# tianhao-stan-wu/LLA-MPC

Hardware: AMD Instinct MI355X
Metric: model-rollouts/sec (N_models x H steps) per control tick; wall-clock per plan() call (higher is better)
Workload: dtype f64

## Files before the change

### __graft_entry__.py

```python
import os
import subprocess
import sys

REPO = os.path.dirname(os.path.abspath(__file__))
PKG_ROOT = os.path.join(REPO, "lla-mpc_amd")
CSRC = os.path.join(PKG_ROOT, "csrc")
LIB = os.path.join(PKG_ROOT, "llampc", "_lib", "libllampc_hip.so")


def _paths():
    for p in (REPO, PKG_ROOT):
        if p not in sys.path:
            sys.path.insert(0, p)


SOURCES = ("capi.hip", "capi_xchg.hip", "capi_ctl.hip", "capi_nlp.hip", "kernels.hip", "ctl.hip", "plan_rk4_l4.hip",
           "plan_rk4_l2.hip", "plan_rk4_l1.hip", "plan_euler.hip", "plan_rk6.hip", "nlp.hip")


def build() -> None:
    hipcc = os.environ.get("HIPCC", "/opt/rocm/bin/hipcc")
    os.makedirs(os.path.dirname(LIB), exist_ok=True)
    objdir = os.path.join(PKG_ROOT, "build")
    os.makedirs(objdir, exist_ok=True)
    flags = ["--offload-arch=gfx950", "-O3", "-std=c++17", "-fPIC", "-mllvm", "-disable-machine-licm",
             f"-I{os.path.join(REPO, 'include')}", "-Wall", "-Wno-unused-result"]
    jobs = max(1, min(len(SOURCES), int(os.environ.get("MAX_JOBS", os.cpu_count() or 4))))
    objs, pending = [], []
    for src in SOURCES:
        obj = os.path.join(objdir, src.replace(".hip", ".o"))
        objs.append(obj)
        pending.append([hipcc, *flags, "-c", "-o", obj, os.path.join(CSRC, src)])
    running = []
    while pending or running:
        while pending and len(running) < jobs:
            cmd = pending.pop(0)
            running.append((cmd, subprocess.Popen(cmd)))
        cmd, p = running.pop(0)
        if p.wait() != 0:
            for _, q in running:
                q.wait()
            raise subprocess.CalledProcessError(p.returncode, cmd)
    subprocess.run([hipcc, "--offload-arch=gfx950", "-shared", "-fPIC", "-o", LIB, *objs], check=True)
    _paths()
    import llampc
    import llampc.mpc
    from llampc import _native
    _native.load()


def smoke() -> None:
    _paths()
    import numpy as np
    from llampc.mpc import ModelBank, generate_bank, plan
    from oracle import llampc_oracle as O

    N, W, K, H, C, Ts = 512, 3, 5, 20, 4, 0.02
    bank_p = generate_bank(N, seed=0)
    p = O.orca_params()
    shared = {k: p[k] for k in ("lf", "lr", "mass", "Iz", "Cm1", "Cm2", "Cr0", "Cr2")}
    rng = np.random.RandomState(5)
    xs = [np.array([0.5, -1.0, -0.6, 1.8, 0.05, 0.4])]
    us = rng.uniform([0.2, -0.2], [0.8, 0.2], size=(W + 2, 2))
    v_true = O.Vehicle.from_params(p, Df=p["Df"] * 0.8, Dr=p["Dr"] * 0.8)
    for k in range(W + 1):
# ... 29 lines not shown
```

### lla-mpc_amd/csrc/lookahead_dev.hpp

```cpp
#pragma once
#include "dev_stamps.hpp"
#include "dev_wave.hpp"
#include "raceline.hpp"
#include "rollout_dev.hpp"

namespace llampc {

template <int NW = kWaves>
__device__ __forceinline__ void la_publish(const LookaheadLaunch& a, int blk, const Scratch& sc, int par,
                                           double v, int64_t key, int nf) {
  static_assert(NW == kWaves || NW == 8, "4- or 8-wave blocks");
  wave_pick_nl64(v, key);
  const int nfw = wave_sum(nf);
  double* sv = sc.sv + 4 * par;
  int64_t* si = sc.si + 4 * par;
  if ((threadIdx.x & 63) == 0) {
    sv[threadIdx.x >> 6] = v;
    si[threadIdx.x >> 6] = key;
    sc.sn[threadIdx.x >> 6] = nfw;
  }
  __syncthreads();
  if (threadIdx.x == 0) {
    int nfs = sc.sn[0];
#pragma unroll
    for (int w = 1; w < NW; ++w) {
      const bool t = (int)(si[w] != kNoIndex) & (int)less_bf<0>(sv[w], si[w], v, key);
      v = t ? sv[w] : v;
      key = t ? si[w] : key;
      nfs += sc.sn[w];
    }
    if (a.poll) {
      uint64_t* r = a.blk_tag + 5 * (int64_t)blk;
      const uint64_t vb = (uint64_t)__double_as_longlong(v), kb = (uint64_t)key;
      st_wt(&r[0], tag_word(a.seq, (uint32_t)(vb >> 32)));
      st_wt(&r[1], tag_word(a.seq, (uint32_t)vb));
      st_wt(&r[2], tag_word(a.seq, (uint32_t)(kb >> 32)));
      st_wt(&r[3], tag_word(a.seq, (uint32_t)kb));
      st_wt(&r[4], tag_word(a.seq, (uint32_t)nfs));
    } else {
      st_wt(&a.pv[blk], v);
      st_wt(&a.pidx[blk], key);
      st_wt(&a.pnf[blk], nfs);
    }
  }
}

template <int INTEG, bool STAGE, int LPM, int XM, int WQ = 0>
__device__ __forceinline__ void lookahead_block(const LookaheadLaunch& a, int blk, int G, int cpl,
                                                unsigned char* smem, const Scratch& sc) {
  LA_STAMP(blk, 0);
  constexpr int BT = wq_threads(WQ);
  double* sx = reinterpret_cast<double*>(smem + kScratchBytes);
  double* su = sx + 2 * (a.H + 1);
  const int H = a.H, C = a.C;
  const int sub = threadIdx.x % LPM;
  const int cl = threadIdx.x / LPM;
  const int g = cl & (G - 1);
  const int64_t n = (int64_t)blk * (kBlock / (G * LPM)) + cl / G;
  const bool live = n < a.n;
  const int mpb = kBlock / (G * LPM);
  const int soff = (XM && mpb < kBlock) ? mpb : 0;
  Tire t{};
  if (!WQ && live) t = load_tire(a.params, a.n, n);
  double x0[6];
#pragma unroll
  for (int m = 0; m < 6; ++m) x0[m] = a.x0[m];
  double* rl_knots = su + (STAGE ? kStageW * C * H : 0);
  double* rl_xy = rl_knots + a.rl.n + kKnotPad;
  if (XM) {
    const int nk = a.rl.n, nseg = a.rl.n - 1, nxy = 8 * nseg;
    const double* gk = a.rl.knots;
    const double* gmu = a.rl.mus;
    double* rl_mus = rl_xy + nxy;
    copy_lds<4>(rl_knots, nk, [&](int e) { return gk[e]; });
    copy_lds<24>(rl_xy, nxy + a.rl.M, [&](int e) {
      const double* p = e < nxy ? gk + nk + e : gmu + (e - nxy);
      return *p;
    });
    if ((int)threadIdx.x < kKnotPad) rl_knots[nk + threadIdx.x] = __builtin_inf();
    const double s0 = a.xref[0];
    const double L = gk[nseg];
    const double adv = window_adv(a.xref[1], a.xref[2], a.Ts, H, a.rl.vmax);
    const bool bounded = adv < L && s0 >= 0.0 && s0 < L;
    double te = s0 + adv;
    if (te >= L) te -= L;
    __syncthreads();
    RL_STAMP(blk, 0);
    int* rl_sel = reinterpret_cast<int*>(sx);
    for (int i = threadIdx.x; i < nseg; i += kBlock) {
      const double ki = rl_knots[i], kn = rl_knots[i + 1];
      const bool last = i == nseg - 1;
      if ((i == 0 || ki <= s0) && (last || !(kn <= s0))) rl_sel[0] = i;
      if ((i == 0 || ki <= te) && (last || !(kn <= te))) rl_sel[1] = i;
    }
    __syncthreads();
    SpeedWin sw{nullptr, 0, 0};
    const int seg0 = rl_sel[0];
    {
      const int lo = seg0, l2 = rl_sel[1];
// ... 19 lines not shown
        const int drow = kBlock / W, dj = kBlock - drow * W, rows = a.rl.M * 4;
        copy_lds<24>(wl, tot, [&](int) {
          int sg = lo + j;
          if (sg >= nseg) sg -= nseg;
          const double v = gsp[(size_t)(row < rows ? row : rows - 1) * nseg + sg];
          row += drow;
          j += dj;
          if (j >= W) {
            j -= W;
            ++row;
          }
          return v;
        });
        __syncthreads();
      }
    }
    RL_STAMP(blk, 1);
    const int64_t m = (int64_t)blk * mpb + threadIdx.x;
    if ((int)threadIdx.x < mpb && m < a.n) {
      const double mu = (a.params[2 * a.n + m] + a.params[5 * a.n + m]) / (9.81 * a.veh.mass);
      const RacelineK rl = a.rl;
      RaceRef rr;
      rr.init(rl, rl_knots, rl_mus, mu, a.xref[0], a.xref[1], a.xref[2], a.Ts, seg0);
      double2* out = reinterpret_cast<double2*>(a.xref_pm + m * 2 * H);
      for (int k = 0; k < H; ++k) {
        double xr, yr;
        rr.step(rl, rl_knots, rl_xy, sw, xr, yr);
        out[k] = make_double2(xr, yr);
      }
    }
    RL_STAMP(blk, 2);
    __threadfence_block();
    RL_STAMP(blk, 3);
  } else {
    for (int e = threadIdx.x; e <= H; e += BT) {
      sx[2 * e] = a.xref[e];
      sx[2 * e + 1] = a.xref[(H + 1) + e];
    }
  }
  fm::FmK K0;
  if constexpr (!XM) K0 = fm::FmK::load<kLeanLA && INTEG == 0>();
  if (STAGE) {
    const fm::FmK K = [&] {
      if constexpr (XM) return fm::FmK::load();
      else return K0;
    }();
    const FusedK fq0 = make_fused(a.veh, make_stage<1>(a.veh, Tire{}, 0), a.Ts, scaled_yaw(LPM));
    for (int e = (int)threadIdx.x - soff; e < C * H; e += BT - soff) {
      if (e < 0) break;
      const int c = e / H, k = e - c * H;
      const double dl = a.U[2 * e + 1];
      double sd, cd;
      if (fm::sincos_fast_ok(dl)) fm::sincos_fast(dl, &sd, &cd, K);
      else LL_SINCOS(dl, &sd, &cd);
      double* o = su + kStageW * (k * C + c);
      const double ua = a.U[2 * e];
      const double p0 = k ? a.U[2 * e - 2] : a.uprev[0], p1 = k ? a.U[2 * e - 1] : a.uprev[1];
      const double d0 = ua - p0, d1 = dl - p1;
      if (INTEG == 0) {
        const FusedIn fi = fused_in(fq0, Input{ua, dl, sd, cd});
        o[0] = fi.F0;
        o[1] = fi.F1;
        o[2] = fi.hmsd;
        o[3] = fi.hmcd;
        o[4] = fi.c5a;
        o[5] = dl;
      } else {
        o[0] = ua;
        o[1] = dl;
        o[2] = sd;
        o[3] = cd;
      }
      o[6] = act_term(a.cost, d0, d1);
      o[7] = (!a.cost.enforce || input_feasible(a.cost, ua, dl, d0, d1)) ? 1.0 : 0.0;
    }
  }
  __syncthreads();

  CostK q = a.cost;
  VehK veh = a.veh;
  double Ts = a.Ts;
  for (int m = 0; m < 4; ++m) {
    pin_vgpr(q.Q[m]);
    pin_vgpr(q.R[m]);
    pin_vgpr(q.P[m]);
  }
  for (int m = 0; m < 2; ++m) {
    pin_vgpr(q.umin[m]);
    pin_vgpr(q.umax[m]);
    pin_vgpr(q.dmax[m]);
  }
  pin_vgpr(veh.lf);
  pin_vgpr(veh.lr);
  pin_vgpr(veh.mass);
  pin_vgpr(veh.inv_mass);
  pin_vgpr(veh.inv_Iz);
  pin_vgpr(veh.Cm1);
  pin_vgpr(veh.Cm2);
  pin_vgpr(veh.Cr0);
  pin_vgpr(veh.Cr2);
  pin_vgpr(Ts);
  const double up0 = a.uprev[0], up1 = a.uprev[1];

  double bv = __builtin_nan("");
  int64_t bc = kNoIndex;
  int nf = 0;
  LA_STAMP(blk, 1);
  constexpr bool kSplit = (INTEG == 0 && LPM == 4);
  constexpr unsigned kRF = (STAGE ? kRStage : 0u) | (XM ? kRXm : 0u);
  constexpr unsigned kRSplitQ = kSplit ? kRSplit : 0u;
  const bool diagQP = a.cost.Q[1] == 0.0 && a.cost.Q[2] == 0.0 && a.cost.P[1] == 0.0 && a.cost.P[2] == 0.0;
  if constexpr (WQ) {
    static_assert(LPM == 1 && XM == 0, "work queue: LPM 1, shared xref");
    const int mpw = 64 / G;
    const int64_t units = (a.n + mpw - 1) / mpw;
    const int lm = (int)(threadIdx.x & 63) / G;
    uint32_t zoff;
    asm volatile("v_mov_b32 %0, 0" : "=v"(zoff));
    auto issue = [&](uint32_t off) -> uint64_t {
      uint64_t v = 0;
      if ((threadIdx.x & 63) == 0)
        v = __hip_atomic_fetch_add(a.wq + off, (uint64_t)1, __ATOMIC_RELAXED, __HIP_MEMORY_SCOPE_AGENT);
      return v;
    };
    auto take = [&](uint64_t v) -> int64_t {
      const uint32_t lo = (uint32_t)__builtin_amdgcn_readlane((int)(uint32_t)v, 0);
      const uint32_t hi = (uint32_t)__builtin_amdgcn_readlane((int)(uint32_t)(v >> 32), 0);
      return (int64_t)(((uint64_t)hi << 32) | lo);
    };
    double vacc = __builtin_nan("");
    int64_t kacc = kNoIndex;
    int nfacc = 0;
    const fm::FmK K = K0;
#ifdef LLAMPC_STAMPS
    int ju = 0;
// ... 44 lines not shown
        }
      }
      WQ_STAMP(blk, ju, 2);
      const int64_t un = take(nxt);
      if (lv && g == 0) {
        if (a.poll) {
          st_wt(&a.la_tag[nm], tag_word(a.seq, (uint32_t)(__double_as_longlong(mv) >> 32)));
          st_wt(&a.la_tag[a.n + nm], tag_word(a.seq, (uint32_t)__double_as_longlong(mv)));
          st_wt(&a.la_tag[2 * a.n + nm], tag_word(a.seq, (uint32_t)(int32_t)mc));
        } else {
          st_wt(&a.best_cand[nm], (int32_t)mc);
          st_wt(&a.best_cost[nm], mv);
        }
        if (mc != kNoIndex) {
          const int64_t key = (a.goff + nm) * C + mc;
          if (less_bf<0>(mv, key, vacc, kacc)) {
            vacc = mv;
            kacc = key;
          }
        }
      }
      WQ_STAMP(blk, ju, 3);
#ifdef LLAMPC_STAMPS
      ++ju;
#endif
      u = un;
    }
    LA_STAMP(blk, 2);
    la_publish<BT / 64>(a, blk, sc, 0, vacc, kacc, nfacc);
    LA_STAMP(blk, 3);
    return;
  }
  if (live) {
    constexpr bool kScaled = (INTEG == 0 && scaled_yaw(LPM));
    StageK sk = make_stage<LPM>(veh, t, sub, INTEG == 0 ? Ts : 1.0);
    if (kScaled) sk.ch[0].lw = sk.ch[0].lw / Ts;
    if (kScaled && LPM == 1) sk.ch[1].lw = sk.ch[1].lw / Ts;
    if (kScaled && LPM == 4 && sub >= 2) {
      sk.ch[0].lw = 0.0;
      sk.ch[0].sg = 0.0;
      sk.ch[0].B = 0.0;
      sk.ch[0].nsB = 0.0;
    }
    const FusedK fq = make_fused(veh, sk, Ts, kScaled);
    const fm::FmK K = [&] {
      if constexpr (XM) return fm::FmK::load<kLeanLA && INTEG == 0>();
      else return K0;
    }();
    for (int j = 0; j < cpl; ++j) {
      const int c = g + j * G;
      if (c >= C) break;
      bool bad = false;
      double J;
      if (kSplit && diagQP)
        J = rollout<INTEG, LPM, kRF | kRFast | kRSplitQ>(a, c, n, x0, sx, su, veh, t, sk, q, Ts, up0, up1, K, fq, bad);
      else
        J = rollout<INTEG, LPM, kRF | kRFast>(a, c, n, x0, sx, su, veh, t, sk, q, Ts, up0, up1, K, fq, bad);
      if (LPM == 2) {
        const int bi = bad;
        bad = __builtin_amdgcn_mov_dpp(bi, kPair0, 0xF, 0xF, false) |
              __builtin_amdgcn_mov_dpp(bi, kPair1, 0xF, 0xF, false);
      } else if (LPM == 4) {
        int bi = bad;
        bi |= __builtin_amdgcn_mov_dpp(bi, kQuadX1, 0xF, 0xF, false);
        bi |= __builtin_amdgcn_mov_dpp(bi, kQuadX2, 0xF, 0xF, false);
        bad = bi;
      }
      if (__builtin_expect(__any(bad), 0)) {
        bool unused = false;
        if (bad) J = rollout<INTEG, LPM, kRF>(a, c, n, x0, sx, su, veh, t, sk, q, Ts, up0, up1, K, fq, unused);
      }
      if (sub == 0) {
        if (a.cost_out) a.cost_out[n * C + c] = J;
        nf += !isfinite(J);
      }
      if (less_nan_last(J, c, bv, bc)) {
        bv = J;
// ... 54 lines not shown
```

### lla-mpc_amd/csrc/plan_dev.hpp

```cpp
#pragma once
#include <algorithm>

#include "final_dev.hpp"
#include "lookahead_dev.hpp"
#include "lookback_dev.hpp"
#include "peer_dev.hpp"

namespace llampc {

template <int INTEG, bool STAGE, int LPM, int XM, bool PX = false, int WQ = 0>
__device__ __forceinline__ void plan_body(const LookbackLaunch& lb, const LookaheadLaunch& la,
                                          const FinalLaunch& fin, int G, int cpl) {
  extern __shared__ __attribute__((aligned(16))) unsigned char smem[];
  const Scratch sc(smem);
  int* flag = reinterpret_cast<int*>(smem + kFlagOff);
  const bool is_lb = (int)blockIdx.x < fin.nb_lb;
  const int lb_blk = (int)blockIdx.x, la_blk = (int)blockIdx.x - fin.nb_lb;
  if constexpr (wq_threads(WQ) > kBlock) {
    if (is_lb && threadIdx.x >= kBlock) return;
  }
  if (is_lb) {
    lookback_block(lb, lb_blk, sc);
    if (!ticket_last(&fin.tickets[0], (unsigned)fin.nb_lb, flag)) return;
    if (fin.full) {
      lb_final(fin, smem);
      if (fin.host_tag) __threadfence_system();
    }
    if (fin.poll) {
      __syncthreads();
      final_poll(fin, sc);
      if constexpr (PX) peer_finish(fin, smem);
      return;
    }
  } else {
    lookahead_block<INTEG, STAGE, LPM, XM, WQ>(la, la_blk, G, cpl, smem, sc);
    if (fin.poll) return;
    if constexpr (wq_threads(WQ) > kBlock) {
      if (threadIdx.x >= kBlock) return;
    }
  }
  const unsigned expected = (unsigned)fin.nb_la + (fin.nb_lb > 0 ? 1u : 0u);
  if (!ticket_last(&fin.tickets[1], expected, flag)) return;
  final_select(fin, sc);
  if constexpr (PX) peer_finish(fin, smem);
}

template <int INTEG, bool STAGE, int LPM, int XM, bool PX = false, int WQ = 0>
__global__ __launch_bounds__(wq_threads(WQ)) void plan_kernel(LookbackLaunch lb, LookaheadLaunch la,
                                                      FinalLaunch fin, int G, int cpl) {
  plan_body<INTEG, STAGE, LPM, XM, PX, WQ>(lb, la, fin, G, cpl);
}

template <int LPM>
__global__ __launch_bounds__(kBlock) void plan_kernel_inl(LookbackLaunch lb, LookaheadLaunch la,
                                                          FinalLaunch fin, int G, int cpl,
                                                          InlinePack pk) {
  const double* v = pk.v;
  lb.x_prev = v;
  lb.u_prev = v + 6;
  lb.x_now = v + 8;
  la.x0 = v + 8;
  la.uprev = v + 14;
  la.xref = v + 16;
  la.U = v + 16 + 2 * (la.H + 1);
  plan_body<0, true, LPM, 0>(lb, la, fin, G, cpl);
}

constexpr size_t kOneBlockPerCuLds = 82 * 1024;

template <int INTEG, bool STAGE, int PX, int WQ>
static void launch_plan_wq(const LookbackLaunch& lb, const LookaheadLaunch& la, const FinalLaunch& f,
                           int G, int cpl, size_t lds, hipStream_t s) {
  allow_lds(plan_kernel<INTEG, STAGE, 1, 0, PX, WQ>);
  hipLaunchKernelGGL((plan_kernel<INTEG, STAGE, 1, 0, PX, WQ>), dim3(f.nb_lb + f.nb_la), dim3(wq_threads(WQ)),
                     lds, s, lb, la, f, G, cpl);
}

template <int INTEG, bool STAGE, int LPM>
static void launch_plan_t(const LookbackLaunch& lb, const LookaheadLaunch& la, const FinalLaunch& f,
                          int G, int cpl, size_t lds, hipStream_t s, int wq = 0) {
  lds = std::max(lds, kOneBlockPerCuLds);
  if constexpr (INTEG == LLAMPC_RK4 && LPM == 1) {
    if (wq) {
      if constexpr (STAGE) {
        if (wq == 2) {
          if (f.px_G) launch_plan_wq<INTEG, STAGE, 1, 2>(lb, la, f, G, cpl, lds, s);
          else launch_plan_wq<INTEG, STAGE, 0, 2>(lb, la, f, G, cpl, lds, s);
          return;
        }
      }
      if (f.px_G) launch_plan_wq<INTEG, STAGE, 1, 1>(lb, la, f, G, cpl, lds, s);
      else launch_plan_wq<INTEG, STAGE, 0, 1>(lb, la, f, G, cpl, lds, s);
      return;
    }
  }
  if constexpr (INTEG == LLAMPC_RK4) {
    if (f.px_G) {
      allow_lds(plan_kernel<INTEG, STAGE, LPM, 0, true>);
      hipLaunchKernelGGL((plan_kernel<INTEG, STAGE, LPM, 0, true>), dim3(f.nb_lb + f.nb_la), dim3(kBlock), lds,
                         s, lb, la, f, G, cpl);
      return;
    }
  }
  if (la.xref_mode == LLAMPC_XREF_RACELINE) {
    allow_lds(plan_kernel<INTEG, STAGE, LPM, 1>);
    hipLaunchKernelGGL((plan_kernel<INTEG, STAGE, LPM, 1>), dim3(f.nb_lb + f.nb_la), dim3(kBlock), lds, s,
                       lb, la, f, G, cpl);
  } else {
    allow_lds(plan_kernel<INTEG, STAGE, LPM, 0>);
    hipLaunchKernelGGL((plan_kernel<INTEG, STAGE, LPM, 0>), dim3(f.nb_lb + f.nb_la), dim3(kBlock), lds, s,
                       lb, la, f, G, cpl);
  }
}

template <int LPM>
static void launch_plan_inl(const LookbackLaunch& lb, const LookaheadLaunch& la, const FinalLaunch& f,
                            int G, int cpl, size_t lds, hipStream_t s, const InlinePack& pk) {
  lds = std::max(lds, kOneBlockPerCuLds);
  allow_lds(plan_kernel_inl<LPM>);
  hipLaunchKernelGGL((plan_kernel_inl<LPM>), dim3(f.nb_lb + f.nb_la), dim3(kBlock), lds, s, lb, la, f,
                     G, cpl, pk);
}

template <int INTEG, int LPM>
void launch_plan_group(const LookbackLaunch& lb, const LookaheadLaunch& la, const FinalLaunch& f, int G,
                       int cpl, bool stage, size_t lds, hipStream_t s, int wq) {
  if (stage) launch_plan_t<INTEG, true, LPM>(lb, la, f, G, cpl, lds, s, wq);
  else launch_plan_t<INTEG, false, LPM>(lb, la, f, G, cpl, lds, s, wq);
}

template <int LPM>
void launch_plan_inline_group(const LookbackLaunch& lb, const LookaheadLaunch& la, const FinalLaunch& f,
                              int G, int cpl, size_t lds, hipStream_t s, const InlinePack& pk) {
  launch_plan_inl<LPM>(lb, la, f, G, cpl, lds, s, pk);
}

}
```

### lla-mpc_amd/csrc/dev_wave.hpp

```cpp
#pragma once
#include <hip/hip_runtime.h>
#include <stdint.h>

#include "kernels.hpp"

namespace llampc {

namespace {

template <int NAN_FIRST>
__device__ __forceinline__ bool kless(double av, int64_t ai, double bv, int64_t bi) {
  return NAN_FIRST ? less_nan_first(av, ai, bv, bi) : less_nan_last(av, ai, bv, bi);
}

constexpr int kDppXor1 = 0xB1, kDppXor2 = 0x4E, kDppRor4 = 0x124, kDppRor8 = 0x128;
template <int CTRL>
__device__ __forceinline__ int dpp_i(int x) {
  return __builtin_amdgcn_update_dpp(x, x, CTRL, 0xF, 0xF, false);
}
template <int CTRL>
__device__ __forceinline__ double dpp_d(double v) {
  return __hiloint2double(dpp_i<CTRL>(__double2hiint(v)), dpp_i<CTRL>(__double2loint(v)));
}
template <int CTRL>
__device__ __forceinline__ int64_t dpp_l(int64_t v) {
  const uint64_t u = (uint64_t)v;
  const uint64_t lo = (uint32_t)dpp_i<CTRL>((int)(uint32_t)u), hi = (uint32_t)dpp_i<CTRL>((int)(u >> 32));
  return (int64_t)(lo | (hi << 32));
}
__device__ __forceinline__ double readlane_d(double v, int l) {
  return __hiloint2double(__builtin_amdgcn_readlane(__double2hiint(v), l),
                          __builtin_amdgcn_readlane(__double2loint(v), l));
}
__device__ __forceinline__ int64_t readlane_l(int64_t v, int l) {
  const uint64_t u = (uint64_t)v;
  const uint64_t lo = (uint32_t)__builtin_amdgcn_readlane((int)(uint32_t)u, l);
  const uint64_t hi = (uint32_t)__builtin_amdgcn_readlane((int)(u >> 32), l);
  return (int64_t)(lo | (hi << 32));
}

template <int NAN_FIRST, int CTRL>
__device__ __forceinline__ void min_step(double& v, int64_t& i) {
  const double ov = dpp_d<CTRL>(v);
  const int64_t oi = dpp_l<CTRL>(i);
  if (kless<NAN_FIRST>(ov, oi, v, i)) {
    v = ov;
    i = oi;
  }
}

template <int NAN_FIRST>
__device__ __forceinline__ void wave_min(double& v, int64_t& i) {
  min_step<NAN_FIRST, kDppXor1>(v, i);
  min_step<NAN_FIRST, kDppXor2>(v, i);
  min_step<NAN_FIRST, kDppRor4>(v, i);
  min_step<NAN_FIRST, kDppRor8>(v, i);
  double bv = readlane_d(v, 0);
  int64_t bi = readlane_l(i, 0);
#pragma unroll
  for (int r = 16; r < 64; r += 16) {
    const double rv = readlane_d(v, r);
    const int64_t ri = readlane_l(i, r);
    if (kless<NAN_FIRST>(rv, ri, bv, bi)) {
      bv = rv;
      bi = ri;
// ... 60 lines not shown
  int64_t q = (int64_t)((double)key / dc);
  q += (int64_t)((double)(key - q * C) / dc);
  int64_t r = key - q * C;
  if (r < 0) {
    q -= 1;
    r += C;
  } else if (r >= C) {
    q += 1;
    r -= C;
  }
  m = q;
  c = (int32_t)r;
}

__device__ __forceinline__ uint64_t tag_word(uint32_t seq, uint32_t payload) {
  return ((uint64_t)seq << 32) | payload;
}
__device__ __forceinline__ bool tag_ok(uint64_t w, uint32_t seq) { return (uint32_t)(w >> 32) == seq; }
__device__ __forceinline__ uint64_t join_words(uint64_t hi, uint64_t lo) {
  return ((uint64_t)(uint32_t)hi << 32) | (uint32_t)lo;
}

__device__ __forceinline__ int wave_sum(int x) {
  x += dpp_i<kDppXor1>(x);
  x += dpp_i<kDppXor2>(x);
  x += dpp_i<kDppRor4>(x);
  x += dpp_i<kDppRor8>(x);
  return __builtin_amdgcn_readlane(x, 0) + __builtin_amdgcn_readlane(x, 16) +
         __builtin_amdgcn_readlane(x, 32) + __builtin_amdgcn_readlane(x, 48);
}

__device__ __forceinline__ void pin_vgpr(double& x) { asm volatile("" : "+v"(x)); }

}

constexpr int kScratchBytes = 192;
constexpr int kFlagOff = 160;
constexpr int kLateOff = 168;
constexpr int kStageW = 8;
constexpr int kRankBytes = 64 * 8 + 64 * 4 + 256;
constexpr int kWaves = kBlock / 64;
constexpr int kListsPerLane = 8;

struct Scratch {
  double* sv;
  int64_t* si;
  int32_t* sn;
  __device__ explicit Scratch(unsigned char* smem)
      : sv(reinterpret_cast<double*>(smem)),
        si(reinterpret_cast<int64_t*>(smem + 64)),
        sn(reinterpret_cast<int32_t*>(smem + 128)) {}
};

template <int NAN_FIRST>
__device__ __forceinline__ void block_min1(double& v, int64_t& i, const Scratch& s, int& par) {
  wave_min<NAN_FIRST>(v, i);
  double* sv = s.sv + 4 * par;
  int64_t* si = s.si + 4 * par;
  par ^= 1;
  if ((threadIdx.x & 63) == 0) {
    sv[threadIdx.x >> 6] = v;
    si[threadIdx.x >> 6] = i;
  }
  __syncthreads();
  v = sv[0];
  i = si[0];
// ... 22 lines not shown
```

Before: 8.347 billion.

## Preload hot kernel arguments and issue early loads ahead of lookahead setup

The plan kernel signature is reordered so the most-used scalars and pointers come first, and a compiler flag enables kernarg preloading into SGPRs for the plan sources; the remaining launch structs are read through the kernarg segment pointer. Lookahead blocks now issue their tire, x0, uprev and first control loads before the main setup, prefetch the next staged control input inside the stage loop, and defer the xref writes to LDS until after staging. The goal is to hide global-load latency at kernel start and cut kernarg fetch cost, at the price of extra register pressure and reliance on a backend-specific LLVM option.

```diff
diff --git a/__graft_entry__.py b/__graft_entry__.py
--- a/__graft_entry__.py
+++ b/__graft_entry__.py
@@ -30,7 +30,8 @@
     for src in SOURCES:
         obj = os.path.join(objdir, src.replace(".hip", ".o"))
         objs.append(obj)
-        pending.append([hipcc, *flags, "-c", "-o", obj, os.path.join(CSRC, src)])
+        plan = ["-mllvm", "-amdgpu-kernarg-preload-count=16"] if src.startswith("plan_") else []
+        pending.append([hipcc, *flags, *plan, "-c", "-o", obj, os.path.join(CSRC, src)])
     running = []
     while pending or running:
         while pending and len(running) < jobs:
diff --git a/lla-mpc_amd/csrc/lookahead_dev.hpp b/lla-mpc_amd/csrc/lookahead_dev.hpp
--- a/lla-mpc_amd/csrc/lookahead_dev.hpp
+++ b/lla-mpc_amd/csrc/lookahead_dev.hpp
@@ -45,9 +45,49 @@
   }
 }
 
+__device__ __forceinline__ void stage_load(const double* U, int e, int H, double* u) {
+  const int k = e % H;
+  const int ep = k ? e - 1 : e;
+  u[0] = U[2 * e];
+  u[1] = U[2 * e + 1];
+  u[2] = U[2 * ep];
+  u[3] = U[2 * ep + 1];
+}
+
+__device__ __forceinline__ double wave_uniform(double v) {
+  const int64_t b = __double_as_longlong(v);
+  const uint32_t lo = (uint32_t)__builtin_amdgcn_readfirstlane((int)(uint32_t)b);
+  const uint32_t hi = (uint32_t)__builtin_amdgcn_readfirstlane((int)(uint32_t)((uint64_t)b >> 32));
+  return __longlong_as_double((int64_t)(((uint64_t)hi << 32) | lo));
+}
+struct LaEarly {
+  Tire t;
+  double x0[6], up0, up1;
+  double u[4];
+};
+template <bool STAGE, int LPM, int XM, int WQ>
+__device__ __forceinline__ LaEarly la_early(const double* U, const double* uprev, const double* x0,
+                                            const double* params, int64_t n, int H, int C, int G, int blk) {
+  LaEarly ev{};
+  uint32_t z;
+  asm volatile("v_mov_b32 %0, 0" : "=v"(z));
+#pragma unroll
+  for (int m = 0; m < 6; ++m) ev.x0[m] = x0[z + m];
+  ev.up0 = uprev[z];
+  ev.up1 = uprev[z + 1];
+  const int mpb = kBlock / (G * LPM);
+  const int64_t nm = (int64_t)blk * mpb + (int)(threadIdx.x / LPM) / G;
+  if (!WQ) ev.t = load_tire(params, n, nm < n ? nm : n - 1);
+  if (STAGE) {
+    const int e = (int)threadIdx.x - ((XM && mpb < kBlock) ? mpb : 0), last = C * H - 1;
+    stage_load(U, e < 0 ? 0 : (e > last ? last : e), H, ev.u);
+  }
+  return ev;
+}
+
 template <int INTEG, bool STAGE, int LPM, int XM, int WQ = 0>
-__device__ __forceinline__ void lookahead_block(const LookaheadLaunch& a, int blk, int G, int cpl,
-                                                unsigned char* smem, const Scratch& sc) {
+__device__ __forceinline__ void lookahead_block(const LookaheadLaunch& a, const LaEarly& ev, int blk, int G,
+                                                int cpl, unsigned char* smem, const Scratch& sc) {
   LA_STAMP(blk, 0);
   constexpr int BT = wq_threads(WQ);
   double* sx = reinterpret_cast<double*>(smem + kScratchBytes);
@@ -60,11 +100,12 @@
   const bool live = n < a.n;
   const int mpb = kBlock / (G * LPM);
   const int soff = (XM && mpb < kBlock) ? mpb : 0;
-  Tire t{};
-  if (!WQ && live) t = load_tire(a.params, a.n, n);
+  const Tire t = ev.t;
   double x0[6];
 #pragma unroll
-  for (int m = 0; m < 6; ++m) x0[m] = a.x0[m];
+  for (int m = 0; m < 6; ++m) x0[m] = ev.x0[m];
+  double up0 = ev.up0, up1 = ev.up1;
+  double xr0 = 0.0, xr1 = 0.0;
   double* rl_knots = su + (STAGE ? kStageW * C * H : 0);
   double* rl_xy = rl_knots + a.rl.n + kKnotPad;
   if (XM) {
@@ -150,11 +191,9 @@
     RL_STAMP(blk, 2);
     __threadfence_block();
     RL_STAMP(blk, 3);
-  } else {
-    for (int e = threadIdx.x; e <= H; e += BT) {
-      sx[2 * e] = a.xref[e];
-      sx[2 * e + 1] = a.xref[(H + 1) + e];
-    }
+  } else if ((int)threadIdx.x <= H) {
+    xr0 = a.xref[threadIdx.x];
+    xr1 = a.xref[(H + 1) + threadIdx.x];
   }
   fm::FmK K0;
   if constexpr (!XM) K0 = fm::FmK::load<kLeanLA && INTEG == 0>();
@@ -164,16 +203,17 @@
       else return K0;
     }();
     const FusedK fq0 = make_fused(a.veh, make_stage<1>(a.veh, Tire{}, 0), a.Ts, scaled_yaw(LPM));
+    double un[4] = {ev.u[0], ev.u[1], ev.u[2], ev.u[3]};
     for (int e = (int)threadIdx.x - soff; e < C * H; e += BT - soff) {
       if (e < 0) break;
       const int c = e / H, k = e - c * H;
-      const double dl = a.U[2 * e + 1];
+      const double ua = un[0], dl = un[1];
+      const double p0 = k ? un[2] : up0, p1 = k ? un[3] : up1;
+      if (e + (BT - soff) < C * H) stage_load(a.U, e + (BT - soff), H, un);
       double sd, cd;
       if (fm::sincos_fast_ok(dl)) fm::sincos_fast(dl, &sd, &cd, K);
       else LL_SINCOS(dl, &sd, &cd);
       double* o = su + kStageW * (k * C + c);
-      const double ua = a.U[2 * e];
-      const double p0 = k ? a.U[2 * e - 2] : a.uprev[0], p1 = k ? a.U[2 * e - 1] : a.uprev[1];
       const double d0 = ua - p0, d1 = dl - p1;
       if (INTEG == 0) {
         const FusedIn fi = fused_in(fq0, Input{ua, dl, sd, cd});
@@ -193,7 +233,21 @@
       o[7] = (!a.cost.enforce || input_feasible(a.cost, ua, dl, d0, d1)) ? 1.0 : 0.0;
     }
   }
+  if constexpr (!XM) {
+    if ((int)threadIdx.x <= H) {
+      sx[2 * threadIdx.x] = xr0;
+      sx[2 * threadIdx.x + 1] = xr1;
+    }
+    for (int e = threadIdx.x + BT; e <= H; e += BT) {
+      sx[2 * e] = a.xref[e];
+      sx[2 * e + 1] = a.xref[(H + 1) + e];
+    }
+  }
   __syncthreads();
+#pragma unroll
+  for (int m = 0; m < 6; ++m) x0[m] = wave_uniform(x0[m]);
+  up0 = wave_uniform(up0);
+  up1 = wave_uniform(up1);
 
   CostK q = a.cost;
   VehK veh = a.veh;
@@ -218,7 +272,6 @@
   pin_vgpr(veh.Cr0);
   pin_vgpr(veh.Cr2);
   pin_vgpr(Ts);
-  const double up0 = a.uprev[0], up1 = a.uprev[1];
 
   double bv = __builtin_nan("");
   int64_t bc = kNoIndex;
diff --git a/lla-mpc_amd/csrc/plan_dev.hpp b/lla-mpc_amd/csrc/plan_dev.hpp
--- a/lla-mpc_amd/csrc/plan_dev.hpp
+++ b/lla-mpc_amd/csrc/plan_dev.hpp
@@ -8,19 +8,50 @@
 
 namespace llampc {
 
-template <int INTEG, bool STAGE, int LPM, int XM, bool PX = false, int WQ = 0>
-__device__ __forceinline__ void plan_body(const LookbackLaunch& lb, const LookaheadLaunch& la,
-                                          const FinalLaunch& fin, int G, int cpl) {
+struct PlanHot {
+  const double *U, *uprev, *x0, *params;
+  int64_t n;
+  int32_t H, C, nb_lb, G;
+};
+struct PlanRest {
+  LookbackLaunch lb;
+  LookaheadLaunch la;
+  FinalLaunch fin;
+  int32_t cpl;
+};
+static_assert(sizeof(PlanHot) == 56 && alignof(PlanRest) == 8, "PlanRest follows the hot arguments at byte 56");
+#define LLAMPC_PLAN_HOT                                                                           \
+  const double *hot_U, const double *hot_uprev, const double *hot_x0, const double *hot_params,   \
+      int64_t hot_n, int32_t hot_H, int32_t hot_C, int32_t hot_nb_lb, int32_t hot_G
+#define LLAMPC_PLAN_HOT_VALUES PlanHot{hot_U, hot_uprev, hot_x0, hot_params, hot_n, hot_H, hot_C, hot_nb_lb, hot_G}
+
+__device__ __forceinline__ const PlanRest& plan_rest() {
+  auto p = (const __attribute__((address_space(4))) unsigned char*)__builtin_amdgcn_kernarg_segment_ptr();
+  return *(const PlanRest*)(p + sizeof(PlanHot));
+}
+
+template <int INTEG, bool STAGE, int LPM, int XM, bool PX = false, int WQ = 0, bool INL = false>
+__device__ __forceinline__ void plan_body(PlanHot hot, const double* pack = nullptr) {
   extern __shared__ __attribute__((aligned(16))) unsigned char smem[];
   const Scratch sc(smem);
   int* flag = reinterpret_cast<int*>(smem + kFlagOff);
-  const bool is_lb = (int)blockIdx.x < fin.nb_lb;
-  const int lb_blk = (int)blockIdx.x, la_blk = (int)blockIdx.x - fin.nb_lb;
+  const bool is_lb = (int)blockIdx.x < hot.nb_lb;
+  const int lb_blk = (int)blockIdx.x, la_blk = (int)blockIdx.x - hot.nb_lb;
   if constexpr (wq_threads(WQ) > kBlock) {
     if (is_lb && threadIdx.x >= kBlock) return;
   }
   if (is_lb) {
-    lookback_block(lb, lb_blk, sc);
+    const PlanRest& r = plan_rest();
+    const FinalLaunch& fin = r.fin;
+    if constexpr (INL) {
+      LookbackLaunch lb = r.lb;
+      lb.x_prev = pack;
+      lb.u_prev = pack + 6;
+      lb.x_now = pack + 8;
+      lookback_block(lb, lb_blk, sc);
+    } else {
+      lookback_block(r.lb, lb_blk, sc);
+    }
     if (!ticket_last(&fin.tickets[0], (unsigned)fin.nb_lb, flag)) return;
     if (fin.full) {
       lb_final(fin, smem);
@@ -33,12 +64,30 @@
       return;
     }
   } else {
-    lookahead_block<INTEG, STAGE, LPM, XM, WQ>(la, la_blk, G, cpl, smem, sc);
-    if (fin.poll) return;
+    if constexpr (INL) {
+      hot.x0 = pack + 8;
+      hot.uprev = pack + 14;
+      hot.U = pack + 16 + 2 * (hot.H + 1);
+    }
+    const LaEarly ev = la_early<STAGE, LPM, XM, WQ>(hot.U, hot.uprev, hot.x0, hot.params, hot.n, hot.H, hot.C,
+                                                    hot.G, la_blk);
+    const PlanRest& r = plan_rest();
+    LookaheadLaunch la = r.la;
+    la.U = hot.U;
+    la.uprev = hot.uprev;
+    la.x0 = hot.x0;
+    la.params = hot.params;
+    la.n = hot.n;
+    la.H = hot.H;
+    la.C = hot.C;
+    if constexpr (INL) la.xref = pack + 16;
+    lookahead_block<INTEG, STAGE, LPM, XM, WQ>(la, ev, la_blk, hot.G, r.cpl, smem, sc);
+    if (r.fin.poll) return;
     if constexpr (wq_threads(WQ) > kBlock) {
       if (threadIdx.x >= kBlock) return;
     }
   }
+  const FinalLaunch& fin = plan_rest().fin;
   const unsigned expected = (unsigned)fin.nb_la + (fin.nb_lb > 0 ? 1u : 0u);
   if (!ticket_last(&fin.tickets[1], expected, flag)) return;
   final_select(fin, sc);
@@ -46,34 +95,30 @@
 }
 
 template <int INTEG, bool STAGE, int LPM, int XM, bool PX = false, int WQ = 0>
-__global__ __launch_bounds__(wq_threads(WQ)) void plan_kernel(LookbackLaunch lb, LookaheadLaunch la,
-                                                      FinalLaunch fin, int G, int cpl) {
-  plan_body<INTEG, STAGE, LPM, XM, PX, WQ>(lb, la, fin, G, cpl);
+__global__ __launch_bounds__(wq_threads(WQ)) void plan_kernel(LLAMPC_PLAN_HOT, PlanRest) {
+  plan_body<INTEG, STAGE, LPM, XM, PX, WQ>(LLAMPC_PLAN_HOT_VALUES);
 }
 
 template <int LPM>
-__global__ __launch_bounds__(kBlock) void plan_kernel_inl(LookbackLaunch lb, LookaheadLaunch la,
-                                                          FinalLaunch fin, int G, int cpl,
-                                                          InlinePack pk) {
-  const double* v = pk.v;
-  lb.x_prev = v;
-  lb.u_prev = v + 6;
-  lb.x_now = v + 8;
-  la.x0 = v + 8;
-  la.uprev = v + 14;
-  la.xref = v + 16;
-  la.U = v + 16 + 2 * (la.H + 1);
-  plan_body<0, true, LPM, 0>(lb, la, fin, G, cpl);
+__global__ __launch_bounds__(kBlock) void plan_kernel_inl(LLAMPC_PLAN_HOT, PlanRest, InlinePack pk) {
+  plan_body<0, true, LPM, 0, false, 0, true>(LLAMPC_PLAN_HOT_VALUES, pk.v);
 }
 
 constexpr size_t kOneBlockPerCuLds = 82 * 1024;
 
+template <typename KERN, typename... Extra>
+static void launch_plan_k(KERN k, int threads, const LookbackLaunch& lb, const LookaheadLaunch& la,
+                          const FinalLaunch& f, int G, int cpl, size_t lds, hipStream_t s,
+                          const Extra&... extra) {
+  allow_lds(k);
+  hipLaunchKernelGGL(k, dim3(f.nb_lb + f.nb_la), dim3(threads), lds, s, la.U, la.uprev, la.x0, la.params,
+                     la.n, la.H, la.C, f.nb_lb, G, PlanRest{lb, la, f, cpl}, extra...);
+}
+
 template <int INTEG, bool STAGE, int PX, int WQ>
 static void launch_plan_wq(const LookbackLaunch& lb, const LookaheadLaunch& la, const FinalLaunch& f,
                            int G, int cpl, size_t lds, hipStream_t s) {
-  allow_lds(plan_kernel<INTEG, STAGE, 1, 0, PX, WQ>);
-  hipLaunchKernelGGL((plan_kernel<INTEG, STAGE, 1, 0, PX, WQ>), dim3(f.nb_lb + f.nb_la), dim3(wq_threads(WQ)),
-                     lds, s, lb, la, f, G, cpl);
+  launch_plan_k(plan_kernel<INTEG, STAGE, 1, 0, PX, WQ>, wq_threads(WQ), lb, la, f, G, cpl, lds, s);
 }
 
 template <int INTEG, bool STAGE, int LPM>
@@ -96,30 +141,21 @@
   }
   if constexpr (INTEG == LLAMPC_RK4) {
     if (f.px_G) {
-      allow_lds(plan_kernel<INTEG, STAGE, LPM, 0, true>);
-      hipLaunchKernelGGL((plan_kernel<INTEG, STAGE, LPM, 0, true>), dim3(f.nb_lb + f.nb_la), dim3(kBlock), lds,
-                         s, lb, la, f, G, cpl);
+      launch_plan_k(plan_kernel<INTEG, STAGE, LPM, 0, true>, kBlock, lb, la, f, G, cpl, lds, s);
       return;
     }
   }
-  if (la.xref_mode == LLAMPC_XREF_RACELINE) {
-    allow_lds(plan_kernel<INTEG, STAGE, LPM, 1>);
-    hipLaunchKernelGGL((plan_kernel<INTEG, STAGE, LPM, 1>), dim3(f.nb_lb + f.nb_la), dim3(kBlock), lds, s,
-                       lb, la, f, G, cpl);
-  } else {
-    allow_lds(plan_kernel<INTEG, STAGE, LPM, 0>);
-    hipLaunchKernelGGL((plan_kernel<INTEG, STAGE, LPM, 0>), dim3(f.nb_lb + f.nb_la), dim3(kBlock), lds, s,
-                       lb, la, f, G, cpl);
-  }
+  if (la.xref_mode == LLAMPC_XREF_RACELINE)
+    launch_plan_k(plan_kernel<INTEG, STAGE, LPM, 1>, kBlock, lb, la, f, G, cpl, lds, s);
+  else
+    launch_plan_k(plan_kernel<INTEG, STAGE, LPM, 0>, kBlock, lb, la, f, G, cpl, lds, s);
 }
 
 template <int LPM>
 static void launch_plan_inl(const LookbackLaunch& lb, const LookaheadLaunch& la, const FinalLaunch& f,
                             int G, int cpl, size_t lds, hipStream_t s, const InlinePack& pk) {
   lds = std::max(lds, kOneBlockPerCuLds);
-  allow_lds(plan_kernel_inl<LPM>);
-  hipLaunchKernelGGL((plan_kernel_inl<LPM>), dim3(f.nb_lb + f.nb_la), dim3(kBlock), lds, s, lb, la, f,
-                     G, cpl, pk);
+  launch_plan_k(plan_kernel_inl<LPM>, kBlock, lb, la, f, G, cpl, lds, s, pk);
 }
 
 template <int INTEG, int LPM>
```

Result: no change. 8.297 billion (-0.6%).

## Prefetch kernel arguments per cache line and batch lookahead prologue loads

Applied to the files above, without the earlier changes.

The plan kernel now issues one scalar load per 64-byte line of its kernel argument segment up front, so later argument reads hit cache instead of stalling one after another. In the non-XM, non-WQ lookahead path, the prologue is reorganised: x0, uprev, xref and the first staged control inputs are loaded early through vector loads, model setup is hoisted ahead of the barrier, and staging processes four elements per batch so global loads overlap. The aim is to cut serialized latency in a latency-bound, single-tick launch. It relies on inline asm with hardcoded offsets tied to the argument struct sizes and adds register pressure.

```diff
diff --git a/lla-mpc_amd/csrc/dev_wave.hpp b/lla-mpc_amd/csrc/dev_wave.hpp
--- a/lla-mpc_amd/csrc/dev_wave.hpp
+++ b/lla-mpc_amd/csrc/dev_wave.hpp
@@ -31,6 +31,10 @@
 __device__ __forceinline__ double readlane_d(double v, int l) {
   return __hiloint2double(__builtin_amdgcn_readlane(__double2hiint(v), l),
                           __builtin_amdgcn_readlane(__double2loint(v), l));
+}
+__device__ __forceinline__ double readfirstlane_d(double v) {
+  return __hiloint2double(__builtin_amdgcn_readfirstlane(__double2hiint(v)),
+                          __builtin_amdgcn_readfirstlane(__double2loint(v)));
 }
 __device__ __forceinline__ int64_t readlane_l(int64_t v, int l) {
   const uint64_t u = (uint64_t)v;
@@ -157,6 +161,44 @@
 
 __device__ __forceinline__ void pin_vgpr(double& x) { asm volatile("" : "+v"(x)); }
 
+typedef const __attribute__((address_space(4))) unsigned char* KernargPtr;
+constexpr int kArgLines = 15;
+template <int BYTES>
+__device__ __forceinline__ KernargPtr touch_kernargs() {
+  static_assert((BYTES + 63) / 64 == kArgLines, "touch_kernargs: one load per line of the arguments");
+  constexpr int kLast = BYTES - 4;
+  static_assert(kLast >= 64 * (kArgLines - 1) && kLast % 4 == 0, "the last word lies in the last line");
+  uint64_t base = (uint64_t)__builtin_amdgcn_kernarg_segment_ptr();
+  uint32_t d0, d1, d2, d3, d4, d5, d6, d7, d8, d9, d10, d11, d12, d13, d14, d15;
+  asm volatile(
+      "s_load_dword %0, %16, 0x0\n\t"
+      "s_load_dword %1, %16, 0x40\n\t"
+      "s_load_dword %2, %16, 0x80\n\t"
+      "s_load_dword %3, %16, 0xc0\n\t"
+      "s_load_dword %4, %16, 0x100\n\t"
+      "s_load_dword %5, %16, 0x140\n\t"
+      "s_load_dword %6, %16, 0x180\n\t"
+      "s_load_dword %7, %16, 0x1c0\n\t"
+      "s_load_dword %8, %16, 0x200\n\t"
+      "s_load_dword %9, %16, 0x240\n\t"
+      "s_load_dword %10, %16, 0x280\n\t"
+      "s_load_dword %11, %16, 0x2c0\n\t"
+      "s_load_dword %12, %16, 0x300\n\t"
+      "s_load_dword %13, %16, 0x340\n\t"
+      "s_load_dword %14, %16, 0x380\n\t"
+      "s_load_dword %15, %16, %17\n\t"
+      "s_waitcnt lgkmcnt(0)"
+      : "=&s"(d0), "=&s"(d1), "=&s"(d2), "=&s"(d3), "=&s"(d4), "=&s"(d5), "=&s"(d6), "=&s"(d7), "=&s"(d8),
+        "=&s"(d9), "=&s"(d10), "=&s"(d11), "=&s"(d12), "=&s"(d13), "=&s"(d14), "=&s"(d15), "+s"(base)
+      : "i"(kLast)
+      : "memory");
+  return (KernargPtr)base;
+}
+template <typename T>
+__device__ __forceinline__ const T& kernarg_at(KernargPtr p, int off) {
+  return *(const T*)reinterpret_cast<const __attribute__((address_space(4))) T*>(p + off);
+}
+
 }
 
 constexpr int kScratchBytes = 192;
diff --git a/lla-mpc_amd/csrc/lookahead_dev.hpp b/lla-mpc_amd/csrc/lookahead_dev.hpp
--- a/lla-mpc_amd/csrc/lookahead_dev.hpp
+++ b/lla-mpc_amd/csrc/lookahead_dev.hpp
@@ -62,9 +62,12 @@
   const int soff = (XM && mpb < kBlock) ? mpb : 0;
   Tire t{};
   if (!WQ && live) t = load_tire(a.params, a.n, n);
+  constexpr bool kBatch = !XM && !WQ;
   double x0[6];
+  if constexpr (!kBatch) {
 #pragma unroll
-  for (int m = 0; m < 6; ++m) x0[m] = a.x0[m];
+    for (int m = 0; m < 6; ++m) x0[m] = a.x0[m];
+  }
   double* rl_knots = su + (STAGE ? kStageW * C * H : 0);
   double* rl_xy = rl_knots + a.rl.n + kKnotPad;
   if (XM) {
@@ -150,75 +153,154 @@
     RL_STAMP(blk, 2);
     __threadfence_block();
     RL_STAMP(blk, 3);
-  } else {
+  } else if (!kBatch) {
     for (int e = threadIdx.x; e <= H; e += BT) {
       sx[2 * e] = a.xref[e];
       sx[2 * e + 1] = a.xref[(H + 1) + e];
     }
   }
-  fm::FmK K0;
-  if constexpr (!XM) K0 = fm::FmK::load<kLeanLA && INTEG == 0>();
-  if (STAGE) {
-    const fm::FmK K = [&] {
-      if constexpr (XM) return fm::FmK::load();
-      else return K0;
-    }();
-    const FusedK fq0 = make_fused(a.veh, make_stage<1>(a.veh, Tire{}, 0), a.Ts, scaled_yaw(LPM));
-    for (int e = (int)threadIdx.x - soff; e < C * H; e += BT - soff) {
-      if (e < 0) break;
-      const int c = e / H, k = e - c * H;
-      const double dl = a.U[2 * e + 1];
-      double sd, cd;
-      if (fm::sincos_fast_ok(dl)) fm::sincos_fast(dl, &sd, &cd, K);
-      else LL_SINCOS(dl, &sd, &cd);
-      double* o = su + kStageW * (k * C + c);
-      const double ua = a.U[2 * e];
-      const double p0 = k ? a.U[2 * e - 2] : a.uprev[0], p1 = k ? a.U[2 * e - 1] : a.uprev[1];
-      const double d0 = ua - p0, d1 = dl - p1;
-      if (INTEG == 0) {
-        const FusedIn fi = fused_in(fq0, Input{ua, dl, sd, cd});
-        o[0] = fi.F0;
-        o[1] = fi.F1;
-        o[2] = fi.hmsd;
-        o[3] = fi.hmcd;
-        o[4] = fi.c5a;
-        o[5] = dl;
-      } else {
-        o[0] = ua;
-        o[1] = dl;
-        o[2] = sd;
-        o[3] = cd;
-      }
-      o[6] = act_term(a.cost, d0, d1);
-      o[7] = (!a.cost.enforce || input_feasible(a.cost, ua, dl, d0, d1)) ? 1.0 : 0.0;
-    }
-  }
-  __syncthreads();
-
+  auto stage_write = [&](int c, int k, double ua, double dl, double sd, double cd, double p0, double p1,
+                         const FusedK& fq0) {
+    double* o = su + kStageW * (k * C + c);
+    const double d0 = ua - p0, d1 = dl - p1;
+    if (INTEG == 0) {
+      const FusedIn fi = fused_in(fq0, Input{ua, dl, sd, cd});
+      o[0] = fi.F0;
+      o[1] = fi.F1;
+      o[2] = fi.hmsd;
+      o[3] = fi.hmcd;
+      o[4] = fi.c5a;
+      o[5] = dl;
+    } else {
+      o[0] = ua;
+      o[1] = dl;
+      o[2] = sd;
+      o[3] = cd;
+    }
+    o[6] = act_term(a.cost, d0, d1);
+    o[7] = (!a.cost.enforce || input_feasible(a.cost, ua, dl, d0, d1)) ? 1.0 : 0.0;
+  };
   CostK q = a.cost;
   VehK veh = a.veh;
   double Ts = a.Ts;
-  for (int m = 0; m < 4; ++m) {
-    pin_vgpr(q.Q[m]);
-    pin_vgpr(q.R[m]);
-    pin_vgpr(q.P[m]);
-  }
-  for (int m = 0; m < 2; ++m) {
-    pin_vgpr(q.umin[m]);
-    pin_vgpr(q.umax[m]);
-    pin_vgpr(q.dmax[m]);
-  }
-  pin_vgpr(veh.lf);
-  pin_vgpr(veh.lr);
-  pin_vgpr(veh.mass);
-  pin_vgpr(veh.inv_mass);
-  pin_vgpr(veh.inv_Iz);
-  pin_vgpr(veh.Cm1);
-  pin_vgpr(veh.Cm2);
-  pin_vgpr(veh.Cr0);
-  pin_vgpr(veh.Cr2);
-  pin_vgpr(Ts);
-  const double up0 = a.uprev[0], up1 = a.uprev[1];
+  auto pin_consts = [&] {
+    for (int m = 0; m < 4; ++m) {
+      pin_vgpr(q.Q[m]);
+      pin_vgpr(q.R[m]);
+      pin_vgpr(q.P[m]);
+    }
+    for (int m = 0; m < 2; ++m) {
+      pin_vgpr(q.umin[m]);
+      pin_vgpr(q.umax[m]);
+      pin_vgpr(q.dmax[m]);
+    }
+    pin_vgpr(veh.lf);
+    pin_vgpr(veh.lr);
+    pin_vgpr(veh.mass);
+    pin_vgpr(veh.inv_mass);
+    pin_vgpr(veh.inv_Iz);
+    pin_vgpr(veh.Cm1);
+    pin_vgpr(veh.Cm2);
+    pin_vgpr(veh.Cr0);
+    pin_vgpr(veh.Cr2);
+    pin_vgpr(Ts);
+  };
+  constexpr bool kScaled = (INTEG == 0 && scaled_yaw(LPM));
+  StageK sk;
+  FusedK fq;
+  auto model_setup = [&] {
+    sk = make_stage<LPM>(veh, t, sub, INTEG == 0 ? Ts : 1.0);
+    if (kScaled) sk.ch[0].lw = sk.ch[0].lw / Ts;
+    if (kScaled && LPM == 1) sk.ch[1].lw = sk.ch[1].lw / Ts;
+    if (kScaled && LPM == 4 && sub >= 2) {
+      sk.ch[0].lw = 0.0;
+      sk.ch[0].sg = 0.0;
+      sk.ch[0].B = 0.0;
+      sk.ch[0].nsB = 0.0;
+    }
+    fq = make_fused(veh, sk, Ts, kScaled);
+  };
+  fm::FmK K0;
+  double up0, up1;
+  if constexpr (!kBatch) {
+    if constexpr (!XM) K0 = fm::FmK::load<kLeanLA && INTEG == 0>();
+    if (STAGE) {
+      const fm::FmK K = [&] {
+        if constexpr (XM) return fm::FmK::load();
+        else return K0;
+      }();
+      const FusedK fq0 = make_fused(a.veh, make_stage<1>(a.veh, Tire{}, 0), a.Ts, scaled_yaw(LPM));
+      for (int e = (int)threadIdx.x - soff; e < C * H; e += BT - soff) {
+        if (e < 0) break;
+        const int c = e / H, k = e - c * H;
+        const double dl = a.U[2 * e + 1];
+        double sd, cd;
+        if (fm::sincos_fast_ok(dl)) fm::sincos_fast(dl, &sd, &cd, K);
+        else LL_SINCOS(dl, &sd, &cd);
+        const double ua = a.U[2 * e];
+        const double p0 = k ? a.U[2 * e - 2] : a.uprev[0], p1 = k ? a.U[2 * e - 1] : a.uprev[1];
+        stage_write(c, k, ua, dl, sd, cd, p0, p1, fq0);
+      }
+    }
+    __syncthreads();
+    pin_consts();
+    up0 = a.uprev[0];
+    up1 = a.uprev[1];
+  } else {
+    const int CH = C * H, tid = (int)threadIdx.x;
+    uint32_t zoff;
+    asm volatile("v_mov_b32 %0, 0" : "=v"(zoff));
+    const double* gx0 = a.x0 + zoff;
+    const double* gup = a.uprev + zoff;
+    double xv[6];
+#pragma unroll
+    for (int m = 0; m < 6; ++m) xv[m] = gx0[m];
+    const double uv0 = gup[0], uv1 = gup[1];
+    const int ex = tid < H ? tid : H;
+    const double xr0 = a.xref[ex], xr1 = a.xref[(H + 1) + ex];
+    auto stage_load = [&](int e, double& ua, double& dl, double& p0, double& p1) {
+      const int ec = e < CH ? e : CH - 1, ep = ec > 0 ? ec - 1 : 0;
+      ua = a.U[2 * ec];
+      dl = a.U[2 * ec + 1];
+      p0 = a.U[2 * ep];
+      p1 = a.U[2 * ep + 1];
+    };
+    double sua = 0.0, sdl = 0.0, sp0 = 0.0, sp1 = 0.0;
+    if (STAGE) stage_load(tid, sua, sdl, sp0, sp1);
+    K0 = fm::FmK::load<kLeanLA && INTEG == 0>();
+    pin_consts();
+    model_setup();
+    for (int e = tid; e <= H; e += BT) {
+      sx[2 * e] = e == tid ? xr0 : a.xref[e];
+      sx[2 * e + 1] = e == tid ? xr1 : a.xref[(H + 1) + e];
+    }
+#pragma unroll
+    for (int m = 0; m < 6; ++m) x0[m] = readfirstlane_d(xv[m]);
+    up0 = readfirstlane_d(uv0);
+    up1 = readfirstlane_d(uv1);
+    if (STAGE) {
+      const FusedK fq0 = make_fused(a.veh, make_stage<1>(a.veh, Tire{}, 0), a.Ts, scaled_yaw(LPM));
+      auto stage_elem = [&](int e, double ua, double dl, double p0, double p1) {
+        const int c = C == 1 ? 0 : e / H, k = e - c * H;
+        double sd, cd;
+        if (fm::sincos_fast_ok(dl)) fm::sincos_fast(dl, &sd, &cd, K0);
+        else LL_SINCOS(dl, &sd, &cd);
+        stage_write(c, k, ua, dl, sd, cd, k ? p0 : uv0, k ? p1 : uv1, fq0);
+      };
+      if (tid < CH) stage_elem(tid, sua, sdl, sp0, sp1);
+      constexpr int kStageBatch = 4;
+      for (int base = tid + BT; base < CH; base += kStageBatch * BT) {
+        double ua[kStageBatch], dl[kStageBatch], p0[kStageBatch], p1[kStageBatch];
+#pragma unroll
+        for (int j = 0; j < kStageBatch; ++j) stage_load(base + j * BT, ua[j], dl[j], p0[j], p1[j]);
+#pragma unroll
+        for (int j = 0; j < kStageBatch; ++j)
+          if (base + j * BT < CH) stage_elem(base + j * BT, ua[j], dl[j], p0[j], p1[j]);
+      }
+    }
+    asm volatile("" ::"v"(xr0), "v"(xr1), "v"(sua), "v"(sdl), "v"(sp0), "v"(sp1));
+    __syncthreads();
+  }
 
   double bv = __builtin_nan("");
   int64_t bc = kNoIndex;
@@ -329,17 +411,7 @@
     return;
   }
   if (live) {
-    constexpr bool kScaled = (INTEG == 0 && scaled_yaw(LPM));
-    StageK sk = make_stage<LPM>(veh, t, sub, INTEG == 0 ? Ts : 1.0);
-    if (kScaled) sk.ch[0].lw = sk.ch[0].lw / Ts;
-    if (kScaled && LPM == 1) sk.ch[1].lw = sk.ch[1].lw / Ts;
-    if (kScaled && LPM == 4 && sub >= 2) {
-      sk.ch[0].lw = 0.0;
-      sk.ch[0].sg = 0.0;
-      sk.ch[0].B = 0.0;
-      sk.ch[0].nsB = 0.0;
-    }
-    const FusedK fq = make_fused(veh, sk, Ts, kScaled);
+    if constexpr (!kBatch) model_setup();
     const fm::FmK K = [&] {
       if constexpr (XM) return fm::FmK::load<kLeanLA && INTEG == 0>();
       else return K0;
diff --git a/lla-mpc_amd/csrc/plan_dev.hpp b/lla-mpc_amd/csrc/plan_dev.hpp
--- a/lla-mpc_amd/csrc/plan_dev.hpp
+++ b/lla-mpc_amd/csrc/plan_dev.hpp
@@ -45,16 +45,30 @@
   if constexpr (PX) peer_finish(fin, smem);
 }
 
+constexpr int kArgLa = sizeof(LookbackLaunch), kArgFin = kArgLa + sizeof(LookaheadLaunch);
+constexpr int kArgG = kArgFin + sizeof(FinalLaunch), kPlanArgBytes = kArgG + 2 * sizeof(int);
+static_assert(sizeof(LookbackLaunch) % 8 == 0 && sizeof(LookaheadLaunch) % 8 == 0 && sizeof(FinalLaunch) % 8 == 0,
+              "plan kernel arguments: no padding between the launch structs");
+
 template <int INTEG, bool STAGE, int LPM, int XM, bool PX = false, int WQ = 0>
 __global__ __launch_bounds__(wq_threads(WQ)) void plan_kernel(LookbackLaunch lb, LookaheadLaunch la,
                                                       FinalLaunch fin, int G, int cpl) {
-  plan_body<INTEG, STAGE, LPM, XM, PX, WQ>(lb, la, fin, G, cpl);
+  if constexpr (XM || WQ) {
+    plan_body<INTEG, STAGE, LPM, XM, PX, WQ>(lb, la, fin, G, cpl);
+  } else {
+    const KernargPtr kp = touch_kernargs<kPlanArgBytes>();
+    plan_body<INTEG, STAGE, LPM, XM, PX, WQ>(kernarg_at<LookbackLaunch>(kp, 0), kernarg_at<LookaheadLaunch>(kp, kArgLa),
+                                             kernarg_at<FinalLaunch>(kp, kArgFin), kernarg_at<int>(kp, kArgG),
+                                             kernarg_at<int>(kp, kArgG + 4));
+  }
 }
 
 template <int LPM>
-__global__ __launch_bounds__(kBlock) void plan_kernel_inl(LookbackLaunch lb, LookaheadLaunch la,
-                                                          FinalLaunch fin, int G, int cpl,
+__global__ __launch_bounds__(kBlock) void plan_kernel_inl(LookbackLaunch, LookaheadLaunch, FinalLaunch, int, int,
                                                           InlinePack pk) {
+  const KernargPtr kp = touch_kernargs<kPlanArgBytes>();
+  LookbackLaunch lb = kernarg_at<LookbackLaunch>(kp, 0);
+  LookaheadLaunch la = kernarg_at<LookaheadLaunch>(kp, kArgLa);
   const double* v = pk.v;
   lb.x_prev = v;
   lb.u_prev = v + 6;
@@ -63,7 +77,8 @@
   la.uprev = v + 14;
   la.xref = v + 16;
   la.U = v + 16 + 2 * (la.H + 1);
-  plan_body<0, true, LPM, 0>(lb, la, fin, G, cpl);
+  plan_body<0, true, LPM, 0>(lb, la, kernarg_at<FinalLaunch>(kp, kArgFin), kernarg_at<int>(kp, kArgG),
+                             kernarg_at<int>(kp, kArgG + 4));
 }
 
 constexpr size_t kOneBlockPerCuLds = 82 * 1024;
```

New measurement: 8.337 billion before, 8.496 billion after (median of 6 runs). +1.9%, better.
